# zijinxuxu/PDFNet

Hardware: AMD Instinct MI355X
Metric: train-step images/sec @256x256 RGB-D B=32 (higher is better)
Workload: dtype f32

## Files before the change

### include/pdfnet_hip.h

```cpp
#ifndef PDFNET_HIP_H
#define PDFNET_HIP_H
#ifdef __cplusplus
extern "C" {
#endif

#define PDF_E_BADARG (-1)
#define PDF_E_WORKSPACE (-2)
#define PDF_ACT_NONE 0
#define PDF_ACT_RELU 1
#define PDF_ACT_LRELU01 2


int pdf_linear_fwd(const float* x, const float* w, const float* bias, float* y,
                   int M, int N, int K, int ldx, int ldw, int ldy, int act, void* stream);
int pdf_linear_bwd_weight(const float* x, const float* dy, float* dw, float* db, float* ws, long ws_floats,
                          int M, int N, int K, int ldx, int lddy, int accumulate, void* stream);
long pdf_wgrad_workspace_floats(int M, int NI, int NJ);
int pdf_init(void);
int pdf_debug_init_device(void);
int pdf_debug_kernel_timing(int on);
int pdf_set_stats_output(float* part, long cap_floats);
long pdf_stats_result_tiles(void);
long pdf_stats_result_rows(void);
int pdf_set_bn_tile_stats(const float* part, long tiles, long rows_per_tile);
int pdf_debug_kernel_record_count(void);
int pdf_debug_kernel_record(int i, char* name, int cap, double* flops, double* bytes, float* ms);
int pdf_stream_wait(void* waiter, void* signaler);
int pdf_set_gemm_precision(int bf16);
int pdf_debug_gemm_precision(void);
int pdf_debug_last_tile(void);
int pdf_debug_igemm_launches(void);
int pdf_linear_bwd_data(const float* dy, const float* w, float* dx, int M, int N, int K, int lddy, int ldw, int lddx, void* stream);
int pdf_linear_fwd_pair(const float* x, const float* w0, const float* w1, const float* b0, const float* b1, float* y,
                        int M, int N, int K, int ldx, int ldw, int ldy, int act, void* stream);
int pdf_linear_bwd_data_pair(const float* dy, const float* w0, const float* w1, float* dx, int M, int N, int K,
                             int lddy, int ldw, int lddx, void* stream);
int pdf_linear_bwd_weight_pair(const float* x, const float* dy, float* dw0, float* dw1, float* db0, float* db1,
                               float* ws, long ws_floats, int M, int N, int K, int ldx, int lddy, int accumulate, void* stream);

int pdf_conv2d_fwd(const float* x, const float* w, const float* bias, float* y,
                   int N, int H, int W, int Cin, int ldx, int Cout, int KH, int KW,
                   int stride, int pad, int OH, int OW, int ldy, int act, void* stream);
int pdf_conv2d_bwd_data(const float* dy, const float* w, float* dx,
                        int N, int H, int W, int Cin, int lddx, int Cout, int KH, int KW,
                        int stride, int pad, int OH, int OW, int lddy, void* stream);
int pdf_conv2d_bwd_data_add(const float* dy, const float* w, float* dx,
                        int N, int H, int W, int Cin, int lddx, int Cout, int KH, int KW,
                        int stride, int pad, int OH, int OW, int lddy, void* stream);
int pdf_conv2d_bwd_weight(const float* x, const float* dy, float* dw, float* db, float* ws, long ws_floats,
                          int N, int H, int W, int Cin, int ldx, int Cout, int KH, int KW,
                          int stride, int pad, int OH, int OW, int lddy, int accumulate, void* stream);

int pdf_deconv2d_fwd(const float* x, const float* w, const float* bias, float* y,
                     int N, int H, int W, int Cin, int ldx, int Cout, int KH, int KW,
                     int stride, int pad, int OH, int OW, int ldy, void* stream);
int pdf_deconv2d_bwd_data(const float* dy, const float* w, float* dx,
                          int N, int H, int W, int Cin, int lddx, int Cout, int KH, int KW,
                          int stride, int pad, int OH, int OW, int lddy, void* stream);
int pdf_deconv2d_bwd_weight(const float* x, const float* dy, float* dw, float* ws, long ws_floats,
                            int N, int H, int W, int Cin, int ldx, int Cout, int KH, int KW,
                            int stride, int pad, int OH, int OW, int lddy, int accumulate, void* stream);
int pdf_bmm_strided(const float* A, const float* B, float* C, int batch, int M, int N, int K, int RB,
                    long sab, long sar, long sam, long sak, long sbb, long sbr, long sbk, long sbn,
                    long scb, long scm, long scn, int beta, void* stream);


int pdf_knn_ball_group(const float* pts, int ldp, int C, int Bc, int N, int S, int K, float r2,
                       int* idx, float* grouped, int ldg, void* stream);
int pdf_group_bwd(const float* dg, int ldg, const int* idx, float* dpts, int ldd, int C,
                  int Bc, int N, int S, int K, void* stream);
int pdf_gather_sub_fwd(const float* u, int ldu, const float* v, int ldv, const int* idx, int Bc, int N, int S, int K, int C,
                       float* y, int ldy, void* stream);
int pdf_gather_sub_bwd(const float* dy, int lddy, const int* idx, float* du, int ldu, float* dv, int ldv,
                       int Bc, int N, int S, int K, int C, void* stream);
int pdf_invert_index(const int* idx, int Bc, int N, int E, int* start, int* list, int* tmp, void* stream);
int pdf_gather_sub_bwd_sorted(const float* dy, int lddy, const int* start, const int* list, float* du, int ldu, float* dv, int ldv,
                              int Bc, int N, int S, int K, int C, void* stream);
int pdf_gather_rows(const float* feat, int ldf, int C, long HW, const long* ind, long ind_bstride,
                    int B, int M, int R, int shift, float* out, int ldo, void* stream);
int pdf_scatter_rows_add(const float* dout, int ldo, int C, long HW, const long* ind, long ind_bstride,
                         int B, int M, int R, int shift, float* dfeat, int ldf, void* stream);
int pdf_window_op(float* feat, int ldf, int C, int H, int W, const long* ind, long ind_bstride,
                  int B, int M, int r, float* buf, const float* src, int mode, void* stream);
int pdf_nms_top1(const float* hm, int BC, int H, int W, long* ind, float* score, void* stream);
int pdf_maxk_fwd(const float* x, int ldx, int C, long R, int K, float* y, int ldy, int* arg, void* stream);
int pdf_maxk_bwd(const float* dy, int ldy, const int* arg, int C, long R, int K, float* dx, int ldx, void* stream);
int pdf_bn_relu_maxk_fwd(const float* y, int ldy, int C, long R, int K, const float* gamma, const float* beta,
                         float* running_mean, float* running_var, float momentum, float eps, int training,
                         float* out, int ldo, int* arg, float* save_mean, float* save_rstd, float* scale, float* shift,
                         float* ws, void* stream);
int pdf_bn_relu_maxk_bwd(const float* dout, int lddo, const int* arg, const float* y, int ldy, const float* save_mean, const float* save_rstd,
                         const float* gamma, const float* scale, const float* shift, int C, long R, int K,
                         float* dy, int lddy, float* dgamma, float* dbeta, int accumulate, float* ws, void* stream);
long pdf_sa_fused_workspace_floats(int Bc, int S, int K, int C1, int C2, int C3);
int pdf_sa_fused_fwd(const float* u, const float* v, const int* idx, int Bc, int N, int S, int K, int C1, int C2, int C3,
                     const float* w2, const float* b2, const float* w3, const float* b3,
                     const float* gamma1, const float* beta1, const float* gamma2, const float* beta2, const float* gamma3, const float* beta3,
                     float* rmean1, float* rvar1, float* rmean2, float* rvar2, float* rmean3, float* rvar3, float momentum, float eps, int training,
                     float* out, int* arg, float* zsel, float* saved, float* ws, long ws_floats, void* stream);
int pdf_sa_fused_bwd(const float* dout, const float* u, const float* v, const int* idx, int Bc, int N, int S, int K, int C1, int C2, int C3,
                     const float* w2, const float* b2, const float* w3, const float* b3,
                     const float* out, const int* arg, const float* zsel, const float* saved,
                     float* dz1, float* dw2, float* db2, float* dw3, float* db3,
                     float* dgamma1, float* dbeta1, float* dgamma2, float* dbeta2, float* dgamma3, float* dbeta3,
                     float* ws, long ws_floats, void* stream);


long pdf_bn_workspace_floats(int C, long R);
int pdf_bn_train_fwd(const float* x, int ldx, int C, long R, const float* gamma, const float* beta,
                     float* running_mean, float* running_var, float momentum, float eps,
                     const float* res, int ldr, int relu, float* y, int ldy,
                     float* save_mean, float* save_rstd, float* scale, float* shift, float* ws, void* stream);
int pdf_bn_eval_fwd(const float* x, int ldx, int C, long R, const float* gamma, const float* beta,
                    const float* running_mean, const float* running_var, float eps,
// ... 244 lines not shown
```

### pdfnet_amd/build.py

```python
import os
import subprocess
import sys
from concurrent.futures import ThreadPoolExecutor

HERE = os.path.dirname(os.path.abspath(__file__))
CSRC = os.path.join(HERE, "csrc")
LIB = os.path.join(HERE, "libpdfnet_hip.so")
INCLUDE = os.path.join(HERE, "..", "include")
SOURCES = ["gemm.hip", "gemm_dma.hip", "gemm_x3.hip", "winograd.hip", "gemm_bf16.hip", "pointops.hip", "norm.hip", "elementwise.hip", "graph.hip", "meshdec.hip", "meshdec_bf16.hip", "meshdec_x3.hip", "mano.hip", "frontend.hip", "loss.hip", "metrics.hip", "icp.hip", "meshcloud.hip", "render.hip", "safused.hip"]
FLAGS = ["--offload-arch=gfx950", "-O3", "-fPIC", "-std=c++17", "-fvisibility=hidden", "-Wno-unused-result", "-I" + INCLUDE]


def _stale(target, deps):
    if not os.path.exists(target):
        return True
    t = os.path.getmtime(target)
    return any(os.path.getmtime(d) > t for d in deps)


def build(force=False, verbose=True):
    hipcc = os.environ.get("HIPCC", "/opt/rocm/bin/hipcc")
    hdrs = [os.path.join(CSRC, "common.h"), os.path.join(CSRC, "gemm_common.h"), os.path.join(CSRC, "gemm_internal.h"), os.path.join(CSRC, "svd3.h"), os.path.join(CSRC, "icp_common.h"), os.path.join(INCLUDE, "pdfnet_hip.h")]
    objs, jobs = [], []
    for s in SOURCES:
        src = os.path.join(CSRC, s)
        obj = os.path.join(CSRC, s.replace(".hip", ".o"))
        objs.append(obj)
        deps = [src] + hdrs + ([os.path.join(CSRC, "meshdec.hip")] if s in ("meshdec_bf16.hip", "meshdec_x3.hip") else [])
        if force or _stale(obj, deps):
            jobs.append([hipcc] + FLAGS + ["-c", src, "-o", obj])

    def run(cmd):
        if verbose:
            print(" ".join(cmd), flush=True)
        subprocess.check_call(cmd)
    with ThreadPoolExecutor(max_workers=4) as ex:
        list(ex.map(run, jobs))
    if force or jobs or _stale(LIB, objs):
        run([hipcc, "--offload-arch=gfx950", "-shared", "-fPIC", "-o", LIB] + objs)
    return LIB


if __name__ == "__main__":
    print(build(force="--force" in sys.argv))
```

### pdfnet_amd/csrc/gemm.hip

```cpp
#include "common.h"

#include "gemm_common.h"
#include "gemm_internal.h"

PDF_API long pdf_conv2d_winograd_v_offset(int N, int H, int W, int Cin, int Cout, int KH, int KW, int stride, int pad) {
    if (!pdf_internal_wino_eligible(N, H, W, Cin, Cout, KH, KW, stride, pad, 0) || !pdf_internal_wino_wgrad_eligible(N, H, W, Cin, Cout, KH, KW, stride, pad)) return -1;
    return pdf_internal_wino_v_offset(N, H, W, Cin, Cout);
}
PDF_API long pdf_conv2d_winograd_workspace_floats(int N, int H, int W, int Cin, int Cout, int KH, int KW, int stride, int pad, int backward) {
    if (backward == 2) return pdf_internal_wino_wgrad_eligible(N, H, W, Cin, Cout, KH, KW, stride, pad) ? pdf_internal_wino_wgrad_workspace(N, H, W, Cin, Cout) : 0;
    const int Ck = backward ? Cout : Cin, Cn = backward ? Cin : Cout;
    return pdf_internal_wino_eligible(N, H, W, Ck, Cn, KH, KW, stride, pad, backward) ? pdf_internal_wino_workspace(N, H, W, Ck, Cn, backward) : 0;
}

constexpr int WG_ISSUE_AT = 1;
typedef unsigned int u32x4v __attribute__((ext_vector_type(4)));
__device__ __forceinline__ float4 as_f4(const u32x4v& v) { return *reinterpret_cast<const float4*>(&v); }

template <int BM, int BN, int WM, int WN, bool FAST, bool KN, int BKT, bool BUF, bool AFF>
__device__ __forceinline__ void igemm_nt_body(const IGemm& g) {
    constexpr int NT = WM * WN * 64;
    constexpr int BK = BKT, LD = BK + 1;
    constexpr int TM = BM / WM / 32, TN = BN / WN / 32;
    constexpr int TPR = BK / 4, RPP = NT / TPR;
// ... 1270 lines not shown
        else if (g.b_kn) hipLaunchKernelGGL((igemm_halo3x3<true, false>), grid, dim3(256), 0, s, g);
        else hipLaunchKernelGGL((igemm_halo3x3<false, false>), grid, dim3(256), 0, s, g);
        g_last_tile = 128128;
    }
    else if (g.N > 64 && t128 >= env_int(ENV_IG_T128, 600) && !short_k) {
        stat_plan(g, co, 128);
        launch_igemm_tile<128, 128, 2, 2>(g, fast, dim3(cdiv(g.M, 128) * cdiv(g.N, 128), groups), s);
        g_last_tile = 128128;
    }
    else if (g.N <= 64 && (long)cdiv(g.M, 128) * groups >= env_int(ENV_IG_T128, 600))
        stat_plan(g, co, 128), launch_igemm_tile<128, 64, 4, 1>(g, fast, dim3(cdiv(g.M, 128) * cdiv(g.N, 64), groups), s), g_last_tile = 128064;
    else if (fast && (long)cdiv(g.M, 64) * cdiv(g.N, 64) * groups < 96 && g.K >= 512 && env_int(ENV_IG_T32, 1)) {
        stat_plan(g, co, 32);
        launch_igemm_tile<32, 32, 1, 1>(g, fast, dim3(cdiv(g.M, 32) * cdiv(g.N, 32), groups), s), g_last_tile = 32032;
    }
    else
    {
        stat_plan(g, co, 64);
        const dim3 grid(cdiv(g.M, 64) * cdiv(g.N, 64), groups);
        if (fast && g.Cin % 32 == 0 && env_int(ENV_IG_BK32, 1)) launch_igemm_tile<64, 64, 2, 2, 32>(g, fast, grid, s);
        else launch_igemm_tile<64, 64, 2, 2>(g, fast, grid, s);
        g_last_tile = 64064;
    }
    PDF_LAUNCH_CHECK();
    return 0;
}

int pdf_internal_batched_wgemm(const float* P, const float* Q, float* slab, int batch, long gsP, long gsQ, int M, int NI, int NJ, int splits, hipStream_t s) {
    if (M % 16 != 0 || NI % 4 != 0 || NJ % 4 != 0 || splits < 1) return PDF_E_BADARG;
    WGemm g = {};
    g.P = P; g.Q = Q; g.M = M; g.NI = NI; g.Cq = NJ; g.T = 1; g.ldp = NI; g.ldq = NJ; g.ldw = NJ;
    g.H = 1; g.W = M; g.QH = 1; g.QW = M; g.sy = 1; g.sx = 1; g.plain_q = 1;
    g.dy[0] = 0; g.dx[0] = 0; g.wt[0] = 0;
    const int rps = cdiv(cdiv(M, splits), 16) * 16;
    splits = cdiv(M, rps);
    g.rows_per_split = rps;
    g.slab = slab; g.batch = batch; g.gsP = gsP; g.gsQ = gsQ; g.gsW = (long)splits * NI * NJ;
    g.beta = 0; g.wbytes = (unsigned)(4.0 * NI * NJ);
    g.pbytes = (unsigned)(4.0 * M * NI); g.qbytes = (unsigned)(4.0 * M * NJ);
    g.uniform = 2;
    dim3 grid((unsigned)(cdiv(NI, 128) * cdiv(NJ, 128)), (unsigned)splits, (unsigned)batch);
    if (env_int(ENV_WG_BATCH_XCD, 1)) {
        g.bsplits = splits;
        grid = dim3((unsigned)(grid.x * 8 * cdiv(splits * batch, 8)));
    }
    KTimer kt("wgemm_tn_dma<3, true>", 2.0 * batch * M * NI * NJ, 4.0 * batch * ((double)M * (NI + NJ) + (double)splits * NI * NJ), s);
    hipLaunchKernelGGL((wgemm_tn_dma<3, true>), grid, dim3(256), 0, s, g);
    PDF_LAUNCH_CHECK();
    return splits;
}

int pdf_internal_batched_gemm(const float* A, const float* B, float* C, int batch, long gsA, long gsB, long gsC, int M, int N, int K, hipStream_t s) {
    IGemm g = {};
    g.A = A; g.B = B; g.C = C; g.bias = nullptr;
    g.M = M; g.N = N; g.K = K; g.Cin = K; g.lda = K; g.ldb = K; g.ldc = N;
    g.T = 1; g.plain_in = 1; g.plain_out = 1; g.act = 0;
    g.H = 1; g.W = M; g.QH = 1; g.QW = M; g.sy = 1; g.sx = 1;
    g.batch = batch; g.gsA = gsA; g.gsB = gsB; g.gsC = gsC;
    if (g_gemm_bf16) return PDF_E_BADARG;
    return launch_igemm(g, s, batch);
}

PDF_API long pdf_deconv2d_x3_workspace_floats(int N, int H, int W, int Cin, int Cout, int KH, int KW, int stride, int pad, int backward) {
    return g_gemm_bf16 ? 0 : pdf_internal_x3_deconv_workspace(N, H, W, Cin, Cout, KH, KW, stride, pad, backward);
}
static void conv_taps(IGemm& g, int KH, int KW, int pad, int dil) {
    g.T = KH * KW;
    for (int ky = 0; ky < KH; ++ky)
        for (int kx = 0; kx < KW; ++kx) {
            int t = ky * KW + kx;
            g.dy[t] = (int)(ky * dil - pad); g.dx[t] = (int)(kx * dil - pad); g.wt[t] = t;
        }
}

static IGemm linear_desc(const float* x, const float* w, const float* bias, float* y,
                         int M, int N, int K, int ldx, int ldw, int ldy, int act) {
    IGemm g = {};
    g.A = x; g.B = w; g.C = y; g.bias = bias;
    g.M = M; g.N = N; g.K = K; g.Cin = K; g.lda = ldx; g.ldb = ldw; g.ldc = ldy;
    g.T = 1; g.plain_in = 1; g.plain_out = 1; g.act = act;
    g.H = 1; g.W = M; g.QH = 1; g.QW = M; g.sy = 1; g.sx = 1;
    return g;
}
static int pdf_linear_fwd_impl(const float* x, const float* w, const float* bias, float* y,
                           int M, int N, int K, int ldx, int ldw, int ldy, int act, void* stream, PdfCallOpts& co) {
    hipStream_t s = (hipStream_t)stream;
    IGemm g = linear_desc(x, w, bias, y, M, N, K, ldx, ldw, ldy, act);
    g.A16 = co.op0_bf16; g.B16 = co.op1_bf16;
    g.a_scale = co.in_scale; g.a_shift = co.in_shift;
    return launch_igemm(g, s, 1, &co);
}
PDF_API int pdf_linear_fwd_x(const float* x, const float* w, const float* bias, float* y,
                           int M, int N, int K, int ldx, int ldw, int ldy, int act, void* stream, PdfCallOpts* opts) {
    return pdf_call_x(opts, pdf_linear_fwd_impl, x, w, bias, y, M, N, K, ldx, ldw, ldy, act, stream);
}
PDF_API int pdf_linear_fwd(const float* x, const float* w, const float* bias, float* y,
                           int M, int N, int K, int ldx, int ldw, int ldy, int act, void* stream) {
    return pdf_call_plain(pdf_linear_fwd_impl, x, w, bias, y, M, N, K, ldx, ldw, ldy, act, stream);
}

static int pdf_linear_fwd_pair_impl(const float* x, const float* w0, const float* w1, const float* b0, const float* b1, float* y,
                                int M, int N, int K, int ldx, int ldw, int ldy, int act, void* stream, PdfCallOpts& co) {
    hipStream_t s = (hipStream_t)stream;
    IGemm g = linear_desc(x, w0, b0, y, M, N, K, ldx, ldw, ldy, act);
    g.B1 = w1; g.bias1 = b1; g.gsA = (long)M * ldx; g.gsC = (long)M * ldy;
    return launch_igemm(g, s, 2);
}
PDF_API int pdf_linear_fwd_pair_x(const float* x, const float* w0, const float* w1, const float* b0, const float* b1, float* y,
                                int M, int N, int K, int ldx, int ldw, int ldy, int act, void* stream, PdfCallOpts* opts) {
    return pdf_call_x(opts, pdf_linear_fwd_pair_impl, x, w0, w1, b0, b1, y, M, N, K, ldx, ldw, ldy, act, stream);
}
PDF_API int pdf_linear_fwd_pair(const float* x, const float* w0, const float* w1, const float* b0, const float* b1, float* y,
                                int M, int N, int K, int ldx, int ldw, int ldy, int act, void* stream) {
    return pdf_call_plain(pdf_linear_fwd_pair_impl, x, w0, w1, b0, b1, y, M, N, K, ldx, ldw, ldy, act, stream);
}

static int pdf_linear_bwd_data_impl(const float* dy, const float* w, float* dx, int M, int N, int K, int lddy, int ldw, int lddx,
                                void* stream, PdfCallOpts& co) {
    hipStream_t s = (hipStream_t)stream;
    IGemm g = linear_desc(dy, w, nullptr, dx, M, K, N, lddy, ldw, lddx, 0);
    g.b_kn = 1; g.btap = 0;
    g.A16 = co.op0_bf16; g.B16 = co.op1_bf16;
    if (ldw == K) { g.B16T = co.op1_bf16_t; g.ldbT = N; }
    return launch_igemm(g, s);
}
PDF_API int pdf_linear_bwd_data_x(const float* dy, const float* w, float* dx, int M, int N, int K, int lddy, int ldw, int lddx,
                                void* stream, PdfCallOpts* opts) {
    return pdf_call_x(opts, pdf_linear_bwd_data_impl, dy, w, dx, M, N, K, lddy, ldw, lddx, stream);
}
PDF_API int pdf_linear_bwd_data(const float* dy, const float* w, float* dx, int M, int N, int K, int lddy, int ldw, int lddx,
                                void* stream) {
    return pdf_call_plain(pdf_linear_bwd_data_impl, dy, w, dx, M, N, K, lddy, ldw, lddx, stream);
}

static int pdf_linear_bwd_data_pair_impl(const float* dy, const float* w0, const float* w1, float* dx, int M, int N, int K,
                                     int lddy, int ldw, int lddx, void* stream, PdfCallOpts& co) {
    hipStream_t s = (hipStream_t)stream;
    IGemm g = linear_desc(dy, w0, nullptr, dx, M, K, N, lddy, ldw, lddx, 0);
    g.b_kn = 1; g.btap = 0;
    g.B1 = w1; g.bias1 = nullptr; g.gsA = (long)M * lddy; g.gsC = (long)M * lddx;
    return launch_igemm(g, s, 2);
}
PDF_API int pdf_linear_bwd_data_pair_x(const float* dy, const float* w0, const float* w1, float* dx, int M, int N, int K,
                                     int lddy, int ldw, int lddx, void* stream, PdfCallOpts* opts) {
    return pdf_call_x(opts, pdf_linear_bwd_data_pair_impl, dy, w0, w1, dx, M, N, K, lddy, ldw, lddx, stream);
}
PDF_API int pdf_linear_bwd_data_pair(const float* dy, const float* w0, const float* w1, float* dx, int M, int N, int K,
                                     int lddy, int ldw, int lddx, void* stream) {
    return pdf_call_plain(pdf_linear_bwd_data_pair_impl, dy, w0, w1, dx, M, N, K, lddy, ldw, lddx, stream);
}


template <int CI, int CO, int KH, int KW>
__global__ __launch_bounds__(256) void tiny_conv_fwd_kernel(const float* __restrict__ x, const float* __restrict__ w, const float* __restrict__ bias,
                                                            float* __restrict__ y, int N, int H, int W, int ldx, int pad, int OH, int OW, int ldy, int act) {
    __shared__ float ws[CO * KH * KW * CI];
    for (int i = threadIdx.x; i < CO * KH * KW * CI; i += 256) ws[i] = w[i];
    __syncthreads();
    const long total = (long)N * OH * OW;
    for (long p = blockIdx.x * 256L + threadIdx.x; p < total; p += (long)gridDim.x * 256) {
        const int ox = (int)(p % OW), oy = (int)((p / OW) % OH);
        const long n = p / ((long)OW * OH);
        float acc[CO];
#pragma unroll
        for (int c = 0; c < CO; ++c) acc[c] = bias ? bias[c] : 0.f;
#pragma unroll
        for (int ky = 0; ky < KH; ++ky)
#pragma unroll
            for (int kx = 0; kx < KW; ++kx) {
                const int iy = oy + ky - pad, ix = ox + kx - pad;
                if (iy < 0 || iy >= H || ix < 0 || ix >= W) continue;
                const float* xp = x + ((n * H + iy) * W + ix) * ldx;
#pragma unroll
                for (int ci = 0; ci < CI; ++ci) {
                    const float v = xp[ci];
#pragma unroll
                    for (int c = 0; c < CO; ++c) acc[c] = fmaf(v, ws[((c * KH + ky) * KW + kx) * CI + ci], acc[c]);
                }
            }
        float* yp = y + p * ldy;
#pragma unroll
        for (int c = 0; c < CO; ++c) {
            float v = acc[c];
            if (act == 1) v = fmaxf(v, 0.f); else if (act == 2) v = v > 0.f ? v : 0.1f * v;
            yp[c] = v;
        }
    }
}
template <int CI, int CO, int KH, int KW>
__global__ __launch_bounds__(256) void tiny_conv_wgrad_kernel(const float* __restrict__ x, const float* __restrict__ dy, float* __restrict__ part,
                                                              int N, int H, int W, int ldx, int pad, int OH, int OW, int lddy) {
    constexpr int NW = CO * KH * KW * CI;
    __shared__ float red[4][NW];
    float acc[NW];
#pragma unroll
    for (int i = 0; i < NW; ++i) acc[i] = 0.f;
    const long total = (long)N * OH * OW;
    for (long p = blockIdx.x * 256L + threadIdx.x; p < total; p += (long)gridDim.x * 256) {
        const int ox = (int)(p % OW), oy = (int)((p / OW) % OH);
        const long n = p / ((long)OW * OH);
        float g[CO];
#pragma unroll
        for (int c = 0; c < CO; ++c) g[c] = dy[p * lddy + c];
#pragma unroll
        for (int ky = 0; ky < KH; ++ky)
#pragma unroll
// ... 737 lines not shown
```

### pdfnet_amd/csrc/gemm_common.h

```cpp
#pragma once
#include "common.h"

typedef float f32x16 __attribute__((ext_vector_type(16)));

#define MAX_TAPS 64

struct IGemm {
    const float* A; const float* B; float* C; const float* bias;
    int M, N, K, Cin;
    int lda, ldb;
    int H, W, QH, QW, sy, sx, T;
    int plain_in, plain_out;
    int OH, OW, osy, osx, ooy, oox, ldc;
    int ps_cout, ps_kw;
    int act;
    int b_kn, btap;
    const float* B1; const float* bias1; long gsA, gsC;
    int ksteps; float* part;
    const void* A16; const void* B16; const void* B116;
    int accum;
    float* stat;
    unsigned int abytes, bbytes;
    unsigned int cbytes;
    unsigned short* C16;
// ... 139 lines not shown
    unsigned int pbytes, qbytes;
    unsigned int wbytes;
    int uniform;
    int batch; long gsW;
    int bsplits;
    int dy[MAX_TAPS], dx[MAX_TAPS], wt[MAX_TAPS];
};


__device__ __forceinline__ float* wave_uniform(float* p) {
    const unsigned long long a = (unsigned long long)p;
    const unsigned lo = (unsigned)__builtin_amdgcn_readfirstlane((int)(unsigned)a), hi = (unsigned)__builtin_amdgcn_readfirstlane((int)(unsigned)(a >> 32));
    return reinterpret_cast<float*>(((unsigned long long)hi << 32) | lo);
}

template <int TM, int TN>
__device__ __forceinline__ void wgemm_finish(const WGemm& g, const f32x16 (&acc)[TM][TN], int i0, int j0, int wm, int wn, int lane,
                                             bool bias_thread, float bval, bool rows_whole = false, int split_ = -1, int plane_ = 0) {
    const int grp = g.batch > 0 ? 0 : blockIdx.z, split = split_ >= 0 ? split_ : (int)blockIdx.y;
    float* slabp = g.batch > 0 ? g.slab + (long)(split_ >= 0 ? plane_ : (int)blockIdx.z) * g.gsW : (grp ? g.slab1 : g.slab);
    float* bslabp = grp ? g.bslab1 : g.bslab;
    const int NJ = g.T * g.Cq;
    if (bias_thread) {
        float* bo = bslabp + (long)split * g.NI + i0 + threadIdx.x;
        *bo = g.beta ? *bo + bval : bval;
    }
    float* out = slabp + (long)split * g.NI * g.ldw;
    if (g.wbytes != 0 && rows_whole) {
        const auto rsW = __builtin_amdgcn_make_buffer_rsrc((void*)wave_uniform(out), 0, g.wbytes, 0x00020000);
        const unsigned ldw4 = (unsigned)g.ldw * 4u;
#pragma unroll
        for (int j = 0; j < TN; ++j) {
            const int col = j0 + wn * TN * 32 + j * 32 + (lane & 31);
            const bool cok = col < NJ;
            const int t = cok ? col / g.Cq : 0;
            const int wcol = g.wt[t] * g.Cq + (col - t * g.Cq);
#pragma unroll
            for (int i = 0; i < TM; ++i) {
                const unsigned vo = cok ? (unsigned)((i0 + wm * TM * 32 + i * 32 + 4 * (lane >> 5)) * g.ldw + wcol) * 4u : 0xffffffffu;
                float v[16];
#pragma unroll
                for (int r = 0; r < 16; ++r) v[r] = acc[i][j][r];
                if (g.beta) {
#pragma unroll
                    for (int r = 0; r < 16; ++r)
                        v[r] += __builtin_bit_cast(float, __builtin_amdgcn_raw_buffer_load_b32(rsW, vo, ((r & 3) + 8 * (r >> 2)) * ldw4, 0));
                }
#pragma unroll
                for (int r = 0; r < 16; ++r)
                    __builtin_amdgcn_raw_buffer_store_b32(__builtin_bit_cast(unsigned, v[r]), rsW, vo, ((r & 3) + 8 * (r >> 2)) * ldw4, 0);
            }
        }
    } else {
#pragma unroll
    for (int j = 0; j < TN; ++j) {
        const int col = j0 + wn * TN * 32 + j * 32 + (lane & 31);
        if (col >= NJ) continue;
        const int t = col / g.Cq;
        const int wcol = g.wt[t] * g.Cq + (col - t * g.Cq);
#pragma unroll
        for (int i = 0; i < TM; ++i)
#pragma unroll
            for (int r = 0; r < 16; ++r) {
                const int row = i0 + wm * TM * 32 + i * 32 + (r & 3) + 8 * (r >> 2) + 4 * (lane >> 5);
                if (row < g.NI) {
                    float* o = out + (long)row * g.ldw + wcol;
                    *o = g.beta ? *o + acc[i][j][r] : acc[i][j][r];
                }
            }
    }
    }
}

struct KTimer {
    KTimer(const char* name, double flops, double bytes, hipStream_t s);
    ~KTimer();
    int slot; hipStream_t stream;
};

int launch_igemm_bf16(const IGemm& g, hipStream_t s, int groups);
int igemm_bf16_tile_rows(const IGemm& g, int groups);
int launch_wgemm_bf16(const WGemm& g, int splits, int groups, int small, hipStream_t s);
int launch_igemm_bf16_dma(const IGemm& g, int tile, int variant, int groups, hipStream_t s);
```

### pdfnet_amd/functional.py

```python
import ctypes
import torch
from torch.autograd import Function

from . import hip
from .hip import ptr, ptr_at, stream

ACT_NONE, ACT_RELU, ACT_LRELU = 0, 1, 2
import os as _os

_byref = ctypes.byref
_CallOpts = hip.CallOpts
USE_SIDE_STREAMS = _os.environ.get("PDFNET_SIDE_STREAMS", "1") != "0"
_side = {}


def _record(obj, stream_):
    if torch.is_tensor(obj):
        obj.record_stream(stream_)
        s16 = getattr(obj, '_pdf_bf16', None)
        if s16 is not None:
            s16.record_stream(stream_)
    elif isinstance(obj, (list, tuple)):
        for o in obj:
            _record(o, stream_)
# ... 98 lines not shown


def shadow_t_of(w):
    if not TRANSPOSED_SHADOWS or shadow_of(w) is None:
        return None
    return getattr(w, '_pdf_bf16_t', None)


def new_shadow(t):
    return torch.empty_like(t, dtype=torch.bfloat16) if shadows_on() else None


_bs = _os.environ.get("PDFNET_BF16_STORAGE", "auto")
BF16_STORAGE = 'auto' if _bs == "auto" else _bs != "0"
BF16_STORAGE_MIN_BATCH = int(_os.environ.get("PDFNET_BF16_STORAGE_MIN_BATCH", "32"))


def storage_on(batch=None):
    if not (BF16_SHADOWS and _GEMM_BF16):
        return False
    if BF16_STORAGE == 'auto':
        return batch is not None and batch >= BF16_STORAGE_MIN_BATCH
    return bool(BF16_STORAGE)


def _lazy_bn(t):
    v = getattr(t, '_pdf_lazy', None)
    if v is None or v[3] != t._version:
        return None
    return v[:3]


DEBUG_PHANTOMS = _os.environ.get("PDFNET_DEBUG_PHANTOMS", "0") != "0"


def _stored16(t):
    v = getattr(t, '_pdf_y16', None)
    if v is None:
        return None
    if v[1] != t._version:
        raise RuntimeError("pdfnet_amd: a bf16-storage phantom tensor was modified in place; its fp32 storage holds no value (PDFNET_BF16_STORAGE)")
    return v[0]



def _O(**kw):
    o = None
    for k, v in kw.items():
        if v is not None:
            if o is None:
                o = _CallOpts()
            setattr(o, k, v)
    if o is None:
        return None, None
    return o, _byref(o)


WINOGRAD = _os.environ.get("PDFNET_WINOGRAD", "1") != "0"
WINOGRAD_INFERENCE = _os.environ.get("PDFNET_WINOGRAD_INFERENCE", "0") != "0"
_wino_cache = {}


def _wino_ws(N, H, W, Cin, Cout, KH, KW, stride, pad, backward, dev):
    if not WINOGRAD or _GEMM_BF16 or KH != 3 or KW != 3 or stride != 1 or pad != 1 or Cin < 64 or Cout < 64:
        return None, None
    key = (N, H, W, Cin, Cout, backward)
    n = _wino_cache.get(key)
    if n is None:
        n = _wino_cache[key] = _L().pdf_conv2d_winograd_workspace_floats(N, H, W, Cin, Cout, KH, KW, stride, pad, backward)
    if n <= 0:
        return None, None
    return torch.empty(n, dtype=torch.float32, device=dev), n


X3_DECONV = _os.environ.get("PDFNET_X3_DECONV", "1") != "0"
_x3d_cache = {}


def set_x3(mode):
    _L().pdf_set_x3_mode(-1 if mode is None else int(mode))
    _wino_cache.clear()
    _wino_voff.clear()
    _x3d_cache.clear()


def _x3_deconv_ws(N, H, W, Cin, Cout, KH, KW, stride, pad, backward, dev):
    if not X3_DECONV or _GEMM_BF16 or KH != KW or stride < 2:
        return None, None
    key = (N, H, W, Cin, Cout, KH, stride, pad, backward)
    n = _x3d_cache.get(key)
    if n is None:
        n = _x3d_cache[key] = _L().pdf_deconv2d_x3_workspace_floats(N, H, W, Cin, Cout, KH, KW, stride, pad, backward)
    if n <= 0:
        return None, None
    return torch.empty(n, dtype=torch.float32, device=dev), n


WINOGRAD_KEEP_V = _os.environ.get("PDFNET_WINOGRAD_KEEP_V", "1") != "0"
_wino_voff = {}


def _wino_v_offset(N, H, W, Cin, Cout, KH, KW, stride, pad):
    key = (N, H, W, Cin, Cout, KH, KW, stride, pad)
    off = _wino_voff.get(key)
    if off is None:
        off = _wino_voff[key] = _L().pdf_conv2d_winograd_v_offset(N, H, W, Cin, Cout, KH, KW, stride, pad)
    return off


WINOGRAD_SHARE = _os.environ.get("PDFNET_WINOGRAD_SHARE", "1") != "0"


def share_winograd_input(x):
    if WINOGRAD_SHARE and x is not None and getattr(x, '_pdf_wino_share', None) is None:
        x._pdf_wino_share = {}
    return x


BN_EPILOGUE_STATS = _os.environ.get("PDFNET_BN_EPILOGUE_STATS", "1") != "0"
_be = _os.environ.get("PDFNET_BN_EPILOGUE_STATS_BF16", "auto")
BN_EPILOGUE_STATS_BF16 = 'auto' if _be == "auto" else _be != "0"


def bf16_modes(batch):
    if not _GEMM_BF16:
        return {'gemm': 'fp32'}
    stats = (batch >= BF16_STORAGE_MIN_BATCH) if BN_EPILOGUE_STATS_BF16 == 'auto' else bool(BN_EPILOGUE_STATS_BF16)
    return {'gemm': 'bf16', 'shadows': BF16_SHADOWS, 'conv_to_bn_storage': 'bf16' if storage_on(batch) else 'fp32',
            'bn_statistics': ('fp32 accumulators in the GEMM epilogue' if (stats and BN_EPILOGUE_STATS) else "the BatchNorm's own pass over the stored tensor"),
            'auto_threshold_batch': BF16_STORAGE_MIN_BATCH}


def _stats_request(stats, rows, cols, dev, batch=None):
    if not (stats and BN_EPILOGUE_STATS):
        return None
    if _GEMM_BF16:
        on = (batch is not None and batch >= BF16_STORAGE_MIN_BATCH) if BN_EPILOGUE_STATS_BF16 == 'auto' else bool(BN_EPILOGUE_STATS_BF16)
        if not on:
            return None
    cap = ((rows + 31) // 32) * cols * 2
    return torch.empty(cap, dtype=torch.float32, device=dev)


def _stats_attach(y, part, o):
    if part is None:
        return
    if o.stats_tiles > 0:
        y._pdf_bn_tiles = (part, o.stats_tiles, o.stats_rows, y._version)


def tile_stats_of(x):
    t = getattr(x, '_pdf_bn_tiles', None)
    if t is None or t[3] != x._version:
        return None
    return t


def carry_stats(src, dst):
    t = getattr(src, '_pdf_bn_tiles', None)
    if t is not None and dst.data_ptr() == src.data_ptr():
        dst._pdf_bn_tiles = t
    return dst


class _forced_fp32:

# ... 2355 lines not shown
```

Baseline: 737.5.

## Add persistent row-streaming MFMA GEMM for tall K=64 linear layers

Adds a specialized persistent kernel for linear forward and backward-data GEMMs with very large M, K=64 and N of 64 or 128. The whole weight matrix stays resident in shared memory, and each block streams 128-row tiles of A with a double-buffered register prefetch, using f32 MFMA with fused bias, activation, optional input affine+ReLU and BN stats. It targets the tile-loading overhead and low reuse of the generic implicit GEMM on these skinny shapes. The cost is more code paths and a stricter eligibility gate, with a fallback to the generic path when conditions are not met.

```diff
diff --git a/include/pdfnet_hip.h b/include/pdfnet_hip.h
--- a/include/pdfnet_hip.h
+++ b/include/pdfnet_hip.h
@@ -30,6 +30,8 @@
 int pdf_debug_gemm_precision(void);
 int pdf_debug_last_tile(void);
 int pdf_debug_igemm_launches(void);
+int pdf_set_rows_gemm_mode(int mode);
+int pdf_debug_rows_gemm_mode(void);
 int pdf_linear_bwd_data(const float* dy, const float* w, float* dx, int M, int N, int K, int lddy, int ldw, int lddx, void* stream);
 int pdf_linear_fwd_pair(const float* x, const float* w0, const float* w1, const float* b0, const float* b1, float* y,
                         int M, int N, int K, int ldx, int ldw, int ldy, int act, void* stream);
diff --git a/pdfnet_amd/build.py b/pdfnet_amd/build.py
--- a/pdfnet_amd/build.py
+++ b/pdfnet_amd/build.py
@@ -7,7 +7,7 @@
 CSRC = os.path.join(HERE, "csrc")
 LIB = os.path.join(HERE, "libpdfnet_hip.so")
 INCLUDE = os.path.join(HERE, "..", "include")
-SOURCES = ["gemm.hip", "gemm_dma.hip", "gemm_x3.hip", "winograd.hip", "gemm_bf16.hip", "pointops.hip", "norm.hip", "elementwise.hip", "graph.hip", "meshdec.hip", "meshdec_bf16.hip", "meshdec_x3.hip", "mano.hip", "frontend.hip", "loss.hip", "metrics.hip", "icp.hip", "meshcloud.hip", "render.hip", "safused.hip"]
+SOURCES = ["gemm.hip", "gemm_rows.hip", "gemm_dma.hip", "gemm_x3.hip", "winograd.hip", "gemm_bf16.hip", "pointops.hip", "norm.hip", "elementwise.hip", "graph.hip", "meshdec.hip", "meshdec_bf16.hip", "meshdec_x3.hip", "mano.hip", "frontend.hip", "loss.hip", "metrics.hip", "icp.hip", "meshcloud.hip", "render.hip", "safused.hip"]
 FLAGS = ["--offload-arch=gfx950", "-O3", "-fPIC", "-std=c++17", "-fvisibility=hidden", "-Wno-unused-result", "-I" + INCLUDE]
 
 
diff --git a/pdfnet_amd/csrc/gemm.hip b/pdfnet_amd/csrc/gemm.hip
--- a/pdfnet_amd/csrc/gemm.hip
+++ b/pdfnet_amd/csrc/gemm.hip
@@ -1376,12 +1376,19 @@
     g.H = 1; g.W = M; g.QH = 1; g.QW = M; g.sy = 1; g.sx = 1;
     return g;
 }
+static int rows_gemm(const IGemm& g, hipStream_t s, PdfCallOpts* co) {
+    if (g_gemm_bf16) return 0;
+    const int rc = launch_rows_gemm_nt(g, co, s);
+    if (rc == 1) { ++g_igemm_launches; g_last_tile = ROWS_TILE_CODE + g.N; }
+    return rc;
+}
 static int pdf_linear_fwd_impl(const float* x, const float* w, const float* bias, float* y,
                            int M, int N, int K, int ldx, int ldw, int ldy, int act, void* stream, PdfCallOpts& co) {
     hipStream_t s = (hipStream_t)stream;
     IGemm g = linear_desc(x, w, bias, y, M, N, K, ldx, ldw, ldy, act);
     g.A16 = co.op0_bf16; g.B16 = co.op1_bf16;
     g.a_scale = co.in_scale; g.a_shift = co.in_shift;
+    if (const int rc = rows_gemm(g, s, &co)) return rc < 0 ? -rc : 0;
     return launch_igemm(g, s, 1, &co);
 }
 PDF_API int pdf_linear_fwd_x(const float* x, const float* w, const float* bias, float* y,
@@ -1416,6 +1423,7 @@
     g.b_kn = 1; g.btap = 0;
     g.A16 = co.op0_bf16; g.B16 = co.op1_bf16;
     if (ldw == K) { g.B16T = co.op1_bf16_t; g.ldbT = N; }
+    if (const int rc = rows_gemm(g, s, nullptr)) return rc < 0 ? -rc : 0;
     return launch_igemm(g, s);
 }
 PDF_API int pdf_linear_bwd_data_x(const float* dy, const float* w, float* dx, int M, int N, int K, int lddy, int ldw, int lddx,
diff --git a/pdfnet_amd/csrc/gemm_common.h b/pdfnet_amd/csrc/gemm_common.h
--- a/pdfnet_amd/csrc/gemm_common.h
+++ b/pdfnet_amd/csrc/gemm_common.h
@@ -245,3 +245,5 @@
 int igemm_bf16_tile_rows(const IGemm& g, int groups);
 int launch_wgemm_bf16(const WGemm& g, int splits, int groups, int small, hipStream_t s);
 int launch_igemm_bf16_dma(const IGemm& g, int tile, int variant, int groups, hipStream_t s);
+int launch_rows_gemm_nt(const IGemm& g, PdfCallOpts* co, hipStream_t s);
+#define ROWS_TILE_CODE 2128000
diff --git a/pdfnet_amd/csrc/gemm_rows.hip b/pdfnet_amd/csrc/gemm_rows.hip
--- /dev/null
+++ b/pdfnet_amd/csrc/gemm_rows.hip
@@ -0,0 +1,206 @@
+#include "common.h"
+
+#include "gemm_common.h"
+#include "gemm_internal.h"
+
+#include <cstdio>
+#include <cstdlib>
+
+typedef unsigned int rows_u32x4 __attribute__((ext_vector_type(4)));
+
+#define ROWS_BM 128
+
+struct RowsNT {
+    const float* A; const float* B; float* C; const float* bias;
+    const float* a_scale; const float* a_shift;
+    float* stat;
+    int M, lda, ldb, ldc, act, ntiles;
+    unsigned abytes, cbytes;
+};
+
+template <int K, int N, bool KN, bool AFF>
+__global__ __launch_bounds__(256, 2) void rows_gemm_nt(const RowsNT g) {
+    constexpr int LDW = K + 4, TN = N / 32, KC = K / 8;
+    __shared__ __attribute__((aligned(16))) float Ws[N * LDW];
+    __shared__ __attribute__((aligned(16))) float Ss[AFF ? 2 * K : 4];
+    __shared__ float Sm[2][4 * N * 3];
+
+    const int tid = threadIdx.x, lane = tid & 63, wave = tid >> 6, n = lane & 31, h = lane >> 5;
+    const int G = gridDim.x;
+    const auto rsA = __builtin_amdgcn_make_buffer_rsrc((void*)g.A, 0, g.abytes, 0x00020000);
+    const auto rsC = __builtin_amdgcn_make_buffer_rsrc((void*)g.C, 0, g.cbytes, 0x00020000);
+    const unsigned lda4 = (unsigned)g.lda * 4u, ldc4 = (unsigned)g.ldc * 4u;
+
+    auto gload = [&](int t, float4 (&a)[KC]) {
+        const int row = t * ROWS_BM + wave * 32 + n;
+        const bool ok = t < g.ntiles && row < g.M;
+        const unsigned base = (unsigned)row * lda4 + (unsigned)h * 16u;
+#pragma unroll
+        for (int c = 0; c < KC; ++c) {
+            const rows_u32x4 v = __builtin_amdgcn_raw_buffer_load_b128(rsA, ok ? base + (unsigned)c * 32u : 0xffffffffu, 0, 0);
+            a[c] = *reinterpret_cast<const float4*>(&v);
+        }
+    };
+
+    float4 a0[KC], a1[KC];
+    gload(blockIdx.x, a0);
+
+    if constexpr (!KN) {
+        for (int i = tid; i < N * K / 4; i += 256) {
+            const int r = i / (K / 4), k4 = (i % (K / 4)) * 4;
+            *reinterpret_cast<float4*>(&Ws[r * LDW + k4]) = *reinterpret_cast<const float4*>(g.B + (long)r * g.ldb + k4);
+        }
+    } else {
+        for (int i = tid; i < N * K / 4; i += 256) {
+            const int k = i / (N / 4), n4 = (i % (N / 4)) * 4;
+            const float4 v = *reinterpret_cast<const float4*>(g.B + (long)k * g.ldb + n4);
+            Ws[(n4 + 0) * LDW + k] = v.x; Ws[(n4 + 1) * LDW + k] = v.y; Ws[(n4 + 2) * LDW + k] = v.z; Ws[(n4 + 3) * LDW + k] = v.w;
+        }
+    }
+    if constexpr (AFF) {
+        for (int i = tid; i < K; i += 256) { Ss[i] = g.a_scale[i]; Ss[K + i] = g.a_shift[i]; }
+    }
+    float bv[TN];
+#pragma unroll
+    for (int j = 0; j < TN; ++j) bv[j] = g.bias != nullptr ? g.bias[j * 32 + n] : 0.f;
+    const bool do_stat = g.stat != nullptr;
+    __syncthreads();
+
+    int par = 0;
+    auto tile = [&](int t, float4 (&a)[KC]) {
+        if constexpr (AFF) {
+#pragma unroll
+            for (int c = 0; c < KC; ++c) {
+                const float4 sc = *reinterpret_cast<const float4*>(&Ss[8 * c + 4 * h]), sh = *reinterpret_cast<const float4*>(&Ss[K + 8 * c + 4 * h]);
+                a[c].x = fmaxf(fmaf(a[c].x, sc.x, sh.x), 0.f); a[c].y = fmaxf(fmaf(a[c].y, sc.y, sh.y), 0.f);
+                a[c].z = fmaxf(fmaf(a[c].z, sc.z, sh.z), 0.f); a[c].w = fmaxf(fmaf(a[c].w, sc.w, sh.w), 0.f);
+            }
+        }
+        f32x16 acc[TN];
+#pragma unroll
+        for (int j = 0; j < TN; ++j)
+#pragma unroll
+            for (int r = 0; r < 16; ++r) acc[j][r] = 0.f;
+#pragma unroll
+        for (int c = 0; c < KC; ++c) {
+            float4 b[TN];
+#pragma unroll
+            for (int j = 0; j < TN; ++j) b[j] = *reinterpret_cast<const float4*>(&Ws[(j * 32 + n) * LDW + 8 * c + 4 * h]);
+#pragma unroll
+            for (int j = 0; j < TN; ++j) acc[j] = __builtin_amdgcn_mfma_f32_32x32x2f32(a[c].x, b[j].x, acc[j], 0, 0, 0);
+#pragma unroll
+            for (int j = 0; j < TN; ++j) acc[j] = __builtin_amdgcn_mfma_f32_32x32x2f32(a[c].y, b[j].y, acc[j], 0, 0, 0);
+#pragma unroll
+            for (int j = 0; j < TN; ++j) acc[j] = __builtin_amdgcn_mfma_f32_32x32x2f32(a[c].z, b[j].z, acc[j], 0, 0, 0);
+#pragma unroll
+            for (int j = 0; j < TN; ++j) acc[j] = __builtin_amdgcn_mfma_f32_32x32x2f32(a[c].w, b[j].w, acc[j], 0, 0, 0);
+        }
+        const int m0 = t * ROWS_BM + wave * 32;
+        const bool whole = (t + 1) * ROWS_BM <= g.M;
+        StatAcc st[TN];
+#pragma unroll
+        for (int j = 0; j < TN; ++j) {
+            st[j] = StatAcc{0.f, 0.f, 0.f, 0.f};
+            const int col = j * 32 + n;
+            float v[16];
+#pragma unroll
+            for (int r = 0; r < 16; ++r) v[r] = acc[j][r] + bv[j];
+            if (g.act == 1) {
+#pragma unroll
+                for (int r = 0; r < 16; ++r) v[r] = fmaxf(v[r], 0.f);
+            } else if (g.act == 2) {
+#pragma unroll
+                for (int r = 0; r < 16; ++r) v[r] = v[r] > 0.f ? v[r] : 0.1f * v[r];
+            }
+            if (whole) {
+                const unsigned vo = (unsigned)((m0 + 4 * h) * g.ldc + col) * 4u;
+#pragma unroll
+                for (int r = 0; r < 16; ++r)
+                    __builtin_amdgcn_raw_buffer_store_b32(__builtin_bit_cast(unsigned, v[r]), rsC, vo, ((r & 3) + 8 * (r >> 2)) * ldc4, 0);
+                if (do_stat) {
+                    st[j].s = v[0];
+#pragma unroll
+                    for (int r = 0; r < 16; ++r) { const float d = v[r] - st[j].s; st[j].a += d; st[j].b = fmaf(d, d, st[j].b); }
+                    st[j].n = 16.f;
+                }
+            } else {
+#pragma unroll
+                for (int r = 0; r < 16; ++r) {
+                    const int row = m0 + (r & 3) + 8 * (r >> 2) + 4 * h;
+                    const bool rok = row < g.M;
+                    __builtin_amdgcn_raw_buffer_store_b32(__builtin_bit_cast(unsigned, v[r]), rsC, rok ? (unsigned)(row * g.ldc + col) * 4u : 0xffffffffu, 0, 0);
+                    if (do_stat && rok) stat_add(st[j], v[r]);
+                }
+            }
+        }
+        if (do_stat) {
+            stat_finish<TN, 4, 1, N>(st, Sm[par], g.stat, t, 0, N, wave, 0, lane, tid);
+            par ^= 1;
+        }
+    };
+
+    for (int t = blockIdx.x; t < g.ntiles; t += 2 * G) {
+        gload(t + G, a1);
+        tile(t, a0);
+        if (t + G >= g.ntiles) break;
+        gload(t + 2 * G, a0);
+        tile(t + G, a1);
+    }
+}
+
+#define ROWS_MIN_M 131072
+static int g_rows_mode = -1;
+static int rows_mode() {
+    static const int env = getenv("PDF_ROWS_GEMM") ? (atoi(getenv("PDF_ROWS_GEMM")) != 0) : 1;
+    return g_rows_mode < 0 ? env : g_rows_mode;
+}
+PDF_API int pdf_set_rows_gemm_mode(int mode) { g_rows_mode = mode < 0 ? -1 : (mode > 2 ? 2 : mode); return 0; }
+PDF_API int pdf_debug_rows_gemm_mode(void) { return rows_mode(); }
+
+static int rows_grid(int ntiles, int per_cu) {
+    static int cus = 0;
+    if (cus == 0) {
+        int dev = 0, v = 0;
+        if (hipGetDevice(&dev) != hipSuccess || hipDeviceGetAttribute(&v, hipDeviceAttributeMultiprocessorCount, dev) != hipSuccess || v <= 0) v = 256;
+        cus = v;
+    }
+    return ntiles < per_cu * cus ? ntiles : per_cu * cus;
+}
+
+static bool rows_aligned16(const void* p) { return (reinterpret_cast<uintptr_t>(p) & 15) == 0; }
+
+template <int K, int N>
+static void rows_nt_launch(const RowsNT& r, bool kn, bool aff, hipStream_t s) {
+    char nm[48];
+    snprintf(nm, sizeof nm, "rows_gemm_nt<%d, %d, %s, %s>", K, N, kn ? "true" : "false", aff ? "true" : "false");
+    KTimer kt(nm, 2.0 * r.M * N * K, 4.0 * ((double)r.M * K + (double)N * K + (double)r.M * N), s);
+    const dim3 grid(rows_grid(r.ntiles, N == 64 ? 4 : 3));
+    if (kn) hipLaunchKernelGGL((rows_gemm_nt<K, N, true, false>), grid, dim3(256), 0, s, r);
+    else if (aff) hipLaunchKernelGGL((rows_gemm_nt<K, N, false, true>), grid, dim3(256), 0, s, r);
+    else hipLaunchKernelGGL((rows_gemm_nt<K, N, false, false>), grid, dim3(256), 0, s, r);
+}
+
+int launch_rows_gemm_nt(const IGemm& g, PdfCallOpts* co, hipStream_t s) {
+    const int mode = rows_mode();
+    if (mode == 0 || (mode == 1 && g.M < ROWS_MIN_M)) return 0;
+    if (g.M <= 0 || g.T != 1 || !g.plain_in || !g.plain_out || g.ps_cout != 0 || g.accum || g.C16 != nullptr || g.A == nullptr || g.batch != 0 || g.ksteps != 0) return 0;
+    if (g.K != 64 || (g.N != 64 && g.N != 128) || g.Cin != g.K) return 0;
+    if (mode == 1 && !(g.N == 64 || (!g.b_kn && (co == nullptr || co->stats_out == nullptr)))) return 0;
+    if (g.lda % 4 != 0 || g.ldb % 4 != 0 || g.lda < g.K || g.ldc < g.N || g.ldb < (g.b_kn ? g.N : g.K) || !rows_aligned16(g.A) || !rows_aligned16(g.B)) return 0;
+    if (g.b_kn && (g.btap != 0 || g.wt[0] != 0 || g.a_scale != nullptr)) return 0;
+    const double aext = 4.0 * ((double)(g.M - 1) * g.lda + g.K), cext = 4.0 * ((double)(g.M - 1) * g.ldc + g.N);
+    if (aext >= 4294967000.0 || cext >= 4294967000.0) return 0;
+    RowsNT r = {};
+    r.A = g.A; r.B = g.B; r.C = g.C; r.bias = g.bias; r.a_scale = g.a_scale; r.a_shift = g.a_shift;
+    r.M = g.M; r.lda = g.lda; r.ldb = g.ldb; r.ldc = g.ldc; r.act = g.act; r.ntiles = cdiv(g.M, ROWS_BM);
+    r.abytes = (unsigned)aext; r.cbytes = (unsigned)cext;
+    if (co != nullptr && co->stats_out != nullptr && (long)r.ntiles * g.N * 2 <= co->stats_cap) {
+        r.stat = co->stats_out;
+        co->stats_tiles = r.ntiles; co->stats_rows = ROWS_BM;
+    }
+    const bool kn = g.b_kn != 0, aff = g.a_scale != nullptr;
+    if (g.N == 64) rows_nt_launch<64, 64>(r, kn, aff, s);
+    else rows_nt_launch<64, 128>(r, kn, aff, s);
+    if (hipError_t e = hipGetLastError()) return -(int)e;
+    return 1;
+}
diff --git a/pdfnet_amd/functional.py b/pdfnet_amd/functional.py
--- a/pdfnet_amd/functional.py
+++ b/pdfnet_amd/functional.py
@@ -204,6 +204,10 @@
     _wino_cache.clear()
     _wino_voff.clear()
     _x3d_cache.clear()
+
+
+def set_rows_gemm(mode):
+    _L().pdf_set_rows_gemm_mode(-1 if mode is None else int(mode))
 
 
 def _x3_deconv_ws(N, H, W, Cin, Cout, KH, KW, stride, pad, backward, dev):
```

Result: slower. 717.0 (-2.8%).
